# pkuyzy/TLC-GNN

Hardware: AMD Instinct MI355X
Metric: persistence-images/sec + LP-forward edges/sec, PubMed-scale, 1/2/4/8 GPU (higher is better)
Workload: dtype f64; 1 GPU

## Files before the change

tlc-gnn_amd/csrc/ext1_dc.h:

```cpp
#pragma once

#ifndef TLC_DC_MIN_POS
#define TLC_DC_MIN_POS 160
#endif
#ifndef TLC_DC_MIN_POS_SHARED
#define TLC_DC_MIN_POS_SHARED 320
#endif
#define TLC_DC_MAX_TIE_RUN 64

namespace {

struct DcMem {
    unsigned *Qab, *Pab;
    unsigned short *Qseg, *Qw, *Pseg, *Pw, *Phin;
    unsigned* inT;
    unsigned* best;
    unsigned short *comp, *hook, *labL, *labR;
    int S_cap;
};

__host__ __device__ constexpr size_t dc_bytes(int K, int S_cap) {
    return al16((size_t)K * 8) + 5 * al16((size_t)K * 2) + al16((size_t)((2 * K + 31) / 32) * 4) + al16((size_t)S_cap * 4) +
           4 * al16((size_t)S_cap * 2);
}

__device__ __forceinline__ DcMem dc_carve(unsigned char* base, int K, int S_cap) {
    DcMem D;
    size_t o = 0;
    D.Qab = (unsigned*)(base + o);  o += al16((size_t)K * 4);
    D.Pab = (unsigned*)(base + o);  o += al16((size_t)K * 4);
    D.Qseg = (unsigned short*)(base + o); o += al16((size_t)K * 2);
    D.Qw = (unsigned short*)(base + o);   o += al16((size_t)K * 2);
    D.Pseg = (unsigned short*)(base + o); o += al16((size_t)K * 2);
    D.Pw = (unsigned short*)(base + o);   o += al16((size_t)K * 2);
    D.Phin = (unsigned short*)(base + o); o += al16((size_t)K * 2);
    D.inT = (unsigned*)(base + o);  o += al16((size_t)((2 * K + 31) / 32) * 4);
    D.best = (unsigned*)(base + o); o += al16((size_t)S_cap * 4);
    D.comp = (unsigned short*)(base + o); o += al16((size_t)S_cap * 2);
    D.hook = (unsigned short*)(base + o); o += al16((size_t)S_cap * 2);
    D.labL = (unsigned short*)(base + o); o += al16((size_t)S_cap * 2);
    D.labR = (unsigned short*)(base + o); o += al16((size_t)S_cap * 2);
    D.S_cap = S_cap;
    return D;
}

template <int W>
__device__ __forceinline__ int block_exscan_u16(unsigned short* a, int N, int* wcnt) {
    const int tid = threadIdx.x;
    const int per = (N + W - 1) / W;
    const int lo = tid * per, hi = lo + per < N ? lo + per : N;
    int s = 0;
    for (int i = lo; i < hi; ++i) s += a[i];
    const int inc = tlc_wave_iscan_i32(s);
    if (W > 64) {
        if (tlc_lane() == 63) wcnt[tid >> 6] = inc;
        __syncthreads();
    }
    int before = inc - s, total;
    if (W > 64) {
        int t = 0;
#pragma unroll
        for (int k = 0; k < W / 64; ++k) {
            const int c = wcnt[k];
            if (k < (tid >> 6)) before += c;
            t += c;
        }
        total = t;
    } else {
        total = __builtin_amdgcn_readlane(inc, 63);
    }
    for (int i = lo; i < hi; ++i) {
        const int v = a[i];
        a[i] = (unsigned short)before;
        before += v;
    }
    __syncthreads();
    return total;
}

template <int W>
struct AnyFlag {
    int* slots;
    int turn;
    __device__ __forceinline__ void init(int* three_ints) {
        slots = three_ints; turn = 0;
        if (threadIdx.x < 3) slots[threadIdx.x] = 0;
        __syncthreads();
    }
    __device__ __forceinline__ bool any(bool v) {
        if (W == 64) { __syncthreads(); return __ballot(v) != 0ull; }
        const int sl = turn % 3;
        if (v) slots[sl] = 1;
        __syncthreads();
        const bool r = slots[sl] != 0;
        if (threadIdx.x == 0) slots[(sl + 2) % 3] = 0;
        ++turn;
        return r;
    }
};

__device__ __forceinline__ bool dc_jump4(unsigned short* a, int y) {
    const unsigned c = a[y];
    const unsigned p1 = a[c];
    if (p1 == c) return false;
    const unsigned p2 = a[p1];
    const unsigned p3 = a[p2];
    a[y] = (unsigned short)p3;
    return a[p3] != p3;
}
template <int W>
__device__ __forceinline__ void dc_flatten(unsigned short* a, int S, AnyFlag<W>& af) {
    for (int it = 0; it < 32; ++it) {
        bool more = false;
        for (int y = threadIdx.x; y < S; y += W) more |= dc_jump4(a, y);
        if (!af.any(more)) break;
    }
}
template <int W>
__device__ __forceinline__ void dc_flatten2(unsigned short* a, unsigned short* b, int S, AnyFlag<W>& af) {
    for (int it = 0; it < 32; ++it) {
        bool more = false;
        for (int y = threadIdx.x; y < S; y += W) { more |= dc_jump4(a, y); more |= dc_jump4(b, y); }
        if (!af.any(more)) break;
    }
}

template <int W, class ItemsA, class ItemsB>
__device__ __forceinline__ void dc_components2(unsigned short* labA, unsigned short* labB, int S, const ItemsA& itemsA,
                                               const ItemsB& itemsB, AnyFlag<W>& af) {
    const int tid = threadIdx.x;
    for (int x = tid; x < S; x += W) { labA[x] = (unsigned short)x; labB[x] = (unsigned short)x; }
    __syncthreads();
    for (int round = 0; round < 64; ++round) {
        bool ch = false;
        itemsA([&](unsigned ab) {
            const unsigned ra = labA[ab >> 16], rb = labA[ab & 0xffffu];
            if (ra < rb) { labA[rb] = (unsigned short)ra; ch = true; }
            else if (rb < ra) { labA[ra] = (unsigned short)rb; ch = true; }
        });
        itemsB([&](unsigned ab) {
            const unsigned ra = labB[ab >> 16], rb = labB[ab & 0xffffu];
            if (ra < rb) { labB[rb] = (unsigned short)ra; ch = true; }
            else if (rb < ra) { labB[ra] = (unsigned short)rb; ch = true; }
        });
        if (!af.any(ch)) break;
        dc_flatten2<W>(labA, labB, S, af);
    }
}

struct LdsSrc {
    const unsigned *pn, *ends, *arank, *finb;
    int MMcap;
    __device__ __forceinline__ bool neg(int i, unsigned& ab, unsigned& w, bool& fin) const {
        const unsigned e = pn[MMcap - 1 - i];
        ab = ends[e]; w = arank[e]; fin = ((finb[w >> 5] >> (w & 31)) & 1u) != 0u;
        return true;
    }
    __device__ __forceinline__ void pos(int k, unsigned& ab, unsigned& w, bool& fin) const {
        const unsigned e = pn[k];
        ab = ends[e]; w = arank[e]; fin = ((finb[w >> 5] >> (w & 31)) & 1u) != 0u;
    }
};
struct HandoffSrc {
    const unsigned *par, *key;
    const ull* query;
    __device__ __forceinline__ bool neg(int i, unsigned& ab, unsigned& w, bool& fin) const {
        const unsigned k = key[i];
        if (k == 0u) return false;
        const unsigned pr = par[i];
        ab = ((unsigned)i << 16) | (pr & 0xffffu); w = (k >> 8) - 1u; fin = (pr >> 31) != 0u;
        return true;
    }
    __device__ __forceinline__ void pos(int k, unsigned& ab, unsigned& w, bool& fin) const {
        const ull q = query[k];
        ab = (unsigned)q; w = ((unsigned)(q >> 40)) - 1u; fin = ((q >> 32) & 1ull) != 0ull;
    }
};

template <int W, class Src>
__device__ __forceinline__ bool ext1_dc_solve(const Src& src, int n, int K, int n_neg_items, int* ctl, int* wcnt,
                                              unsigned char* scratch, size_t scratch_bytes, unsigned short* out_hin,
                                              unsigned long long* prof = nullptr) {
    const int tid = threadIdx.x;
    unsigned long long t_prev = prof ? clock64() : 0ull;
#define DC_STAMP(k) do { if (prof && tid == 0) { const unsigned long long _t = clock64(); prof[(k)] += _t - t_prev; t_prev = _t; } } while (0)
    const int S_cap = (n > 2 * K + 2 ? n : 2 * K + 2);
    if (K < 2 || K > 16000 || S_cap > 65000 || dc_bytes(K, S_cap) > scratch_bytes) return false;
    const DcMem D = dc_carve(scratch, K, S_cap);
    int* n_pslot = &ctl[10];
    int* bad = &ctl[11];
    if (tid == 0) { *n_pslot = 0; *bad = 0; }
    AnyFlag<W> af;
    af.init(&ctl[12]);
    dc_components2<W>(D.labL, D.labR, n, [&](auto edge) {
        for (int i = tid; i < n_neg_items; i += W) {
            unsigned ab, w; bool fin;
            if (src.neg(i, ab, w, fin) && fin) edge(ab);
        }
    }, [&](auto) {}, af);
    for (int d = tid; d < K; d += W) D.Pseg[d] = 0xFFFFu;
    __syncthreads();
    for (int i = tid; i < n_neg_items; i += W) {
        unsigned ab, w; bool fin;
        if (src.neg(i, ab, w, fin) && !fin) {
            const int d = atomicAdd(n_pslot, 1);
            if (d < K) {
                const unsigned a = ab >> 16, b = ab & 0xffffu;
                D.Pab[d] = ((unsigned)D.labL[a] << 16) | D.labL[b];
                D.Pw[d] = (unsigned short)w;
                D.Phin[d] = (unsigned short)(a > b ? a : b);
                D.Pseg[d] = 0;
            }
        }
    }
    for (int k = tid; k < K; k += W) {
        unsigned ab, w; bool fin;
        src.pos(k, ab, w, fin);
        D.Qab[k] = ((unsigned)D.labL[ab >> 16] << 16) | D.labL[ab & 0xffffu];
        D.Qw[k] = (unsigned short)w;
        D.Qseg[k] = (unsigned short)(fin ? 0x8000u : 0u);
    }
    __syncthreads();
    DC_STAMP(0);
    int S = n;
    int levels = 0;
    while ((1 << levels) < K) ++levels;
    for (int L = 0; L < levels; ++L) {
        const int n_p = *n_pslot < K ? *n_pslot : K;
        auto mid_of = [&](int j) { return (int)(((long long)(2 * j + 1) * K) >> (L + 1)); };
        for (int x = tid; x < S; x += W) D.comp[x] = (unsigned short)x;
        for (int w = tid; w < (2 * K + 31) / 32; w += W) D.inT[w] = 0u;
        __syncthreads();
        for (int round = 0; round < 48; ++round) {
            for (int x = tid; x < S; x += W) { D.best[x] = 0xFFFFFFFFu; D.hook[x] = 0xFFFFu; }
            __syncthreads();
            bool found = false;
            for (int d = tid; d < n_p; d += W) {
                if (D.Pseg[d] == 0xFFFFu) continue;
                const unsigned ab = D.Pab[d];
                const unsigned ra = D.comp[ab >> 16], rb = D.comp[ab & 0xffffu];
                if (ra != rb) {
                    const unsigned key = ((unsigned)D.Pw[d] << 16) | (unsigned)d;
                    atomicMin(&D.best[ra], key); atomicMin(&D.best[rb], key);
                    found = true;
                }
            }
            for (int k = tid; k < K; k += W) {
                if (k >= mid_of(D.Qseg[k] & 0x7FFF)) continue;
                const unsigned ab = D.Qab[k];
                const unsigned ra = D.comp[ab >> 16], rb = D.comp[ab & 0xffffu];
                if (ra != rb) {
                    const unsigned key = ((unsigned)D.Qw[k] << 16) | (unsigned)(K + k);
                    atomicMin(&D.best[ra], key); atomicMin(&D.best[rb], key);
                    found = true;
                }
            }
            if (!af.any(found)) break;
            for (int x = tid; x < S; x += W) {
                const unsigned key = D.best[x];
                if (key == 0xFFFFFFFFu || D.comp[x] != x) continue;
                const int code = (int)(key & 0xffffu);
                const unsigned ab = code < K ? D.Pab[code] : D.Qab[code - K];
                const unsigned ra = D.comp[ab >> 16], rb = D.comp[ab & 0xffffu];
                const unsigned other = (ra == (unsigned)x) ? rb : ra;
                atomicOr(&D.inT[code >> 5], 1u << (code & 31));
                if (D.best[other] != key || (unsigned)x > other) D.hook[x] = (unsigned short)other;
            }
            __syncthreads();
            for (int x = tid; x < S; x += W)
                if (D.hook[x] != 0xFFFFu) D.comp[x] = D.hook[x];
            __syncthreads();
            dc_flatten<W>(D.comp, S, af);
            if (prof && tid == 0) prof[4] += 1;
        }
        DC_STAMP(1);
        auto in_t = [&](int code) { return ((D.inT[code >> 5] >> (code & 31)) & 1u) != 0u; };
        dc_components2<W>(D.labL, D.labR, S, [&](auto edge) {
            for (int d = tid; d < n_p; d += W)
                if (D.Pseg[d] != 0xFFFFu && in_t(d)) edge(D.Pab[d]);
        }, [&](auto edge) {
            for (int k = tid; k < K; k += W) {
                const unsigned sg = D.Qseg[k];
                if (k < mid_of(sg & 0x7FFF) && (sg & 0x8000u) && in_t(K + k)) edge(D.Qab[k]);
            }
        }, af);
        DC_STAMP(2);
        unsigned short* flag = D.comp;
        for (int x = tid; x < 2 * S; x += W) flag[x] = 0;
        __syncthreads();
        auto child_ab = [&](unsigned ab, bool right) -> unsigned {
            const unsigned a = ab >> 16, b = ab & 0xffffu;
            return right ? (((unsigned)(S + D.labR[a]) << 16) | (unsigned)(S + D.labR[b]))
                         : (((unsigned)D.labL[a] << 16) | (unsigned)D.labL[b]);
        };
        for (int d = tid; d < n_p; d += W) {
            if (D.Pseg[d] == 0xFFFFu) continue;
            const unsigned c = child_ab(D.Pab[d], in_t(d));
            flag[c >> 16] = 1; flag[c & 0xffffu] = 1;
        }
        for (int k = tid; k < K; k += W) {
            const bool left = k < mid_of(D.Qseg[k] & 0x7FFF);
            const unsigned c = child_ab(D.Qab[k], !left);
            flag[c >> 16] = 1; flag[c & 0xffffu] = 1;
            if (left && in_t(K + k) && !(D.Qseg[k] & 0x8000u)) {
                const unsigned c2 = child_ab(D.Qab[k], true);
                flag[c2 >> 16] = 1; flag[c2 & 0xffffu] = 1;
            }
        }
        __syncthreads();
        const int S_next = block_exscan_u16<W>(flag, 2 * S, wcnt);
        if (S_next > S_cap) { if (tid == 0) *bad = 1; __syncthreads(); break; }
        auto renum = [&](unsigned c) -> unsigned { return ((unsigned)flag[c >> 16] << 16) | (unsigned)flag[c & 0xffffu]; };
        for (int d = tid; d < n_p; d += W) {
            const unsigned sg = D.Pseg[d];
            if (sg == 0xFFFFu) continue;
            const bool right = in_t(d);
            D.Pab[d] = renum(child_ab(D.Pab[d], right));
            D.Pseg[d] = (unsigned short)(2 * sg + (right ? 1 : 0));
        }
        for (int k = tid; k < K; k += W) {
            const unsigned sg = D.Qseg[k];
            const int j = (int)(sg & 0x7FFF);
            const unsigned ab = D.Qab[k];
            if (k < mid_of(j)) {
                const bool alive_mid = in_t(K + k);
                if (alive_mid && !(sg & 0x8000u)) {
                    const int d = atomicAdd(n_pslot, 1);
                    if (d < K) {
                        D.Pab[d] = renum(child_ab(ab, true));
                        D.Pw[d] = D.Qw[k];
                        { unsigned qab, qw; bool qf; src.pos(k, qab, qw, qf);
                          D.Phin[d] = (unsigned short)((qab >> 16) > (qab & 0xffffu) ? (qab >> 16) : (qab & 0xffffu)); }
                        D.Pseg[d] = (unsigned short)(2 * j + 1);
                    } else *bad = 1;
                }
                D.Qab[k] = renum(child_ab(ab, false));
                D.Qseg[k] = (unsigned short)((2 * j) | (alive_mid ? 0x8000u : 0u));
            } else {
                D.Qab[k] = renum(child_ab(ab, true));
                D.Qseg[k] = (unsigned short)((2 * j + 1) | (sg & 0x8000u));
            }
        }
        __syncthreads();
        S = S_next;
        DC_STAMP(3);
        if (prof && tid == 0) prof[5] += 1;
        if (*bad) break;
    }
    bool fail = (*bad != 0) || (*n_pslot != K);
    __syncthreads();
    if (!fail) {
        for (int w = tid; w < (K + 31) / 32; w += W) D.inT[w] = 0u;
        __syncthreads();
        for (int d = tid; d < K; d += W) {
            const unsigned sg = D.Pseg[d];
            if (sg == 0xFFFFu) { fail = true; continue; }
            const int k = (int)(((long long)sg * K) >> levels);
            const int k1 = (int)(((long long)(sg + 1) * K) >> levels);
            if (k1 - k != 1 || k >= K) { fail = true; continue; }
            const unsigned old = atomicOr(&D.inT[k >> 5], 1u << (k & 31));
            if ((old >> (k & 31)) & 1u) { fail = true; continue; }
            if (D.Pw[d] <= D.Qw[k]) { fail = true; continue; }
            out_hin[k] = D.Phin[d];
        }
        __syncthreads();
    }
#undef DC_STAMP
    return !af.any(fail);
}

template <int W, typename idx_t>
__device__ __forceinline__ bool fix_desc_ties(Mem<idx_t>& M, int m) {
    const int tid = threadIdx.x;
    constexpr int PER = 8;
    int np_[PER];
    unsigned ne_[PER];
    bool too_long = false;
#pragma unroll
    for (int q = 0; q < PER; ++q) {
        const int pos = tid + q * W;
        np_[q] = -1;
        if (pos < m) {
            const ull k = M.keyS[pos];
            const bool tl = pos > 0 && M.keyS[pos - 1] == k, tr = pos + 1 < m && M.keyS[pos + 1] == k;
            if (tl || tr) {
                int s = pos, t = pos + 1;
                while (s > 0 && M.keyS[s - 1] == k && pos - s <= TLC_DC_MAX_TIE_RUN) --s;
                while (t < m && M.keyS[t] == k && t - pos <= TLC_DC_MAX_TIE_RUN) ++t;
                if (t - s > TLC_DC_MAX_TIE_RUN) too_long = true;
                else {
                    const unsigned e = M.valS[pos];
                    const unsigned ar = M.arank[e];
                    int c = 0;
                    for (int j = s; j < t; ++j) c += (M.arank[M.valS[j]] > ar);
                    np_[q] = s + c;
                    ne_[q] = e;
                }
            }
        }
    }
    const bool bad = block_any<W>(too_long, M.ctl, 0);
    if (!bad) {
#pragma unroll
        for (int q = 0; q < PER; ++q)
            if (np_[q] >= 0) M.valS[np_[q]] = ne_[q];
    }
    __syncthreads();
    return !bad;
}

}
```

tlc-gnn_amd/csrc/pd_pipeline.hip:

```cpp
#include "tlc_common.h"
#include "tlc_kernels.h"
#include "pd_keys.h"

#define TLC_INF_BITS 0x7FF0000000000000ull
#ifdef TLC_PHASE_DEBUG
#define TLC_STAMP(k)                                                                 \
    do {                                                                             \
        if (pc && threadIdx.x == 0) {                                                \
            const unsigned long long _t = clock64();                                 \
            ph[(k)] += _t - t_prev;              \
            t_prev = _t;                                                             \
        }                                                                            \
    } while (0)
#else
#define TLC_STAMP(k) do { } while (0)
#endif
#define TLC_NONE16 0xFFFFu
#ifndef TLC_STOP_AFTER
#define TLC_STOP_AFTER 10
#endif
#define TLC_STOPPED 99

namespace {

// ... 1518 lines not shown
        TLC_STAMP(11);
#ifdef TLC_PHASE_DEBUG
        if (pc && tid == 0) {
            const ull tot = clock64() - t_begin;
            for (int k = 0; k < 12; ++k) if (ph[k]) atomicAdd(&pc[k], ph[k]);
            atomicAdd(&pc[12], tot);
            atomicAdd(&pc[14], 1ull);
            if (atomicMax(&pc[13], tot) < tot) {
                for (int k = 0; k < 12; ++k) pc[16 + k] = ph[k];
                pc[28] = (ull)n; pc[29] = (ull)m;
            }
        }
#endif
        if (status != TLC_ST_OK) acc = 0.0;
        if (!deferred) {
            if (p.out_pi && tid < res2) p.out_pi[(size_t)i * res2 + tid] = acc;
            if (p.out_status && tid == 0) p.out_status[i] = (unsigned char)status;
        }
        __syncthreads();
    } while (HUGE && (wi += (int)gridDim.x) < tier_count);
}

struct SwapLayout {
    size_t o_rec, o_pts, o_ctl, total, table_bytes;
};
__host__ __device__ constexpr SwapLayout make_swap_layout(int NM, int MM) {
    SwapLayout L{};
    size_t o = al16(smax(MM <= 1024 ? swap_table_c_bytes(NM) : swap_table_bytes(NM), (size_t)8 * NM + (size_t)64 * 13 * 8));
    L.table_bytes = o - (size_t)8 * NM;
    L.o_rec = o;  o += 1280;
    L.o_pts = o;  o += al16((size_t)(MM + 2) * 4);
    L.o_ctl = o;  o += 64;
    L.total = o;
    return L;
}

template <int NM, int MM, int W>
__device__ __forceinline__ void swap_subgraph(const TlcPdParams& p, int wi, unsigned char* lds_raw) {
    constexpr SwapLayout L = make_swap_layout(NM, MM);
    const int tid = threadIdx.x;
    const Handoff H = carve_handoff(p.handoff + (size_t)wi * (size_t)p.handoff_stride, NM);
    if (H.hdr[0] == 0) return;
    const int i = wi < p.n_hi ? p.tier_list_hi[wi] : p.tier_list[wi - p.n_hi];
    const int n = H.hdr[1], npos = H.hdr[2], np0 = H.hdr[3], n_up = H.hdr[4];
    const bool any_unreached = H.hdr[5] != 0;
    unsigned* pts = (unsigned*)(lds_raw + L.o_pts);
    int* ctl = (int*)(lds_raw + L.o_ctl);
#ifdef TLC_PHASE_DEBUG
    const ull t_begin = clock64();
#endif
    for (int k = tid; k < np0; k += W) pts[k] = H.pts[k];
    PtsSink sink{pts, ctl};
    if constexpr (MM <= 1024) {
        const SwapTablesC T = carve_swap_c(lds_raw, NM);
        unsigned* recs = (unsigned*)(lds_raw + L.o_rec);
        for (int k = tid; k < n; k += W) {
            const unsigned pr = H.par[k];
            T.pk[k] = ((H.key[k] >> 8) << 16) | (pr == 0xffffffffu ? 0xffffu : (pr & 0xffffu));
            T.slot[k] = 0ull;
        }
        if (tid == 0) { T.pk[NM] = (unsigned)NM; T.slot[NM] = 0ull; }
        __syncthreads();
        if (tid < 64) {
            QueryGlobal qs{H.query, npos, 0u, 0u, 0u, 0u, 0u, 0u};
            const int n_out = ext1_walk_c(T, recs, qs, npos, NM, any_unreached, sink, np0);
            if (tid == 0) ctl[2] = np0 + n_out;
        }
    } else {
        const SwapTables T = carve_swap(lds_raw, NM);
        ull* recs = (ull*)(lds_raw + L.o_rec);
        for (int k = tid; k < n; k += W) {
            const unsigned pr = H.par[k];
            T.par[k] = pr == 0xffffffffu ? pr : (pr & 0x7fffffffu);
            T.key[k] = H.key[k];
            T.mark[k] = 0u;
        }
        if (tid == 0) { T.par[NM] = (unsigned)NM; T.key[NM] = 0u; T.mark[NM] = 0u; }
        __syncthreads();
        if (tid < 64) {
            QueryGlobal qs{H.query, npos, 0u, 0u, 0u, 0u, 0u, 0u};
            const int n_out = ext1_walk(T, recs, qs, npos, NM, any_unreached, sink, (const double*)nullptr, false, np0, nullptr);
            if (tid == 0) ctl[2] = np0 + n_out;
        }
    }
    __syncthreads();
    const int np = ctl[2];
    double* f = (double*)lds_raw;
    for (int k = tid; k < n; k += W) f[k] = H.f[k];
    __syncthreads();
    auto get = [&](int k, double& b, double& d) {
        const unsigned bd = pts[k];
        b = f[bd >> 16];
        d = f[bd & 0xffffu];
    };
    const int res = p.res, res2 = res * res;
    double* table = (double*)(lds_raw + (size_t)8 * NM);
    double acc = 0.0;
    if (p.flags & TLC_PI_ORD0_EXT1) {
        acc = pi_stage<W, true, 64>(table, L.table_bytes, get, 0, n_up, res, acc);
        acc = pi_stage<W, true, 64>(table, L.table_bytes, get, n_up + 1, np, res, acc);
    } else {
        acc = pi_stage<W, true, 64>(table, L.table_bytes, get, 0, np, res, acc);
    }
    if (p.out_pi && tid < res2) p.out_pi[(size_t)i * res2 + tid] = acc;
    if (p.out_status && tid == 0) p.out_status[i] = (unsigned char)TLC_ST_OK;
#ifdef TLC_PHASE_DEBUG
    if (p.phase_cycles && tid == 0) { atomicAdd(&p.phase_cycles[10], clock64() - t_begin); atomicAdd(&p.phase_cycles[12], clock64() - t_begin); }
#endif
    __syncthreads();
}

template <int NM, int MM, bool PLAIN = false>
__global__ __launch_bounds__(64, 4) void tlc_pd_swap_kernel(TlcPdParams p) {
    extern __shared__ __attribute__((aligned(16))) unsigned char lds_raw[];
    if constexpr (PLAIN) { p.flags = 0u; p.res = 5; p.pi_enabled = 1; }
    if (p.abort_flag && *p.abort_flag) return;
    int tier_count = p.tier_count;
    if (p.tier_count_dev) { const int c = *p.tier_count_dev; tier_count = c < tier_count ? c : tier_count; }
    if (tier_count > p.handoff_cap) tier_count = p.handoff_cap;
    if ((int)blockIdx.x < tier_count) swap_subgraph<NM, MM, 64>(p, (int)blockIdx.x, lds_raw);
}

__host__ __device__ constexpr size_t dc_kernel_lds(int NM, int MM) {
    const int KB = NM <= TLC_M_NMAX ? (MM / 8) * 7 : MM / 2;
    const size_t dc = al16(dc_bytes(KB, NM > 2 * KB + 2 ? NM : 2 * KB + 2) + (size_t)MM + 16) + al16((size_t)(MM + 2) * 4) + 256;
    return dc > make_swap_layout(NM, MM).total ? dc : make_swap_layout(NM, MM).total;
}
template <int NM, int MM, int W>
__device__ __forceinline__ void dc_subgraph(const TlcPdParams& p, int wi, unsigned char* lds_raw) {
    constexpr size_t total = dc_kernel_lds(NM, MM);
    constexpr size_t o_pts = total - 256 - al16((size_t)(MM + 2) * 4), o_ctl = total - 256;
    const int tid = threadIdx.x;
    unsigned* pts = (unsigned*)(lds_raw + o_pts);
    int* ctl = (int*)(lds_raw + o_ctl);
    int* wcnt = ctl + 16;
    do {
        const Handoff H = carve_handoff(p.handoff + (size_t)wi * (size_t)p.handoff_stride, NM);
        if (H.hdr[0] == 0 || H.hdr[6] == 0) continue;
        const int i = wi < p.n_hi ? p.tier_list_hi[wi] : p.tier_list[wi - p.n_hi];
        const int n = H.hdr[1], K = H.hdr[2], np0 = H.hdr[3], n_up = H.hdr[4];
        const size_t hin_bytes = al16((size_t)K * 2);
        if (hin_bytes + 16 >= o_pts || np0 + K > MM + 2) { __syncthreads(); swap_subgraph<NM, MM, W>(p, wi, lds_raw); continue; }
        unsigned short* hin = (unsigned short*)(lds_raw + (o_pts - hin_bytes));
        const HandoffSrc src{H.par, H.key, H.query};
        __syncthreads();
#ifdef TLC_PHASE_DEBUG
        unsigned long long prof[8] = {0, 0, 0, 0, 0, 0, 0, 0};
        const unsigned long long t_begin = p.phase_cycles ? clock64() : 0ull;
        const bool ok = ext1_dc_solve<W>(src, n, K, n, ctl, wcnt, lds_raw, o_pts - hin_bytes, hin, p.phase_cycles ? prof : nullptr) && !p.dc_force_fail;
        if (p.phase_cycles && tid == 0) {
            const unsigned long long tot = clock64() - t_begin;
            if (atomicMax(&p.phase_cycles[13], tot) < tot) {
                for (int k = 0; k < 6; ++k) p.phase_cycles[16 + k] = prof[k];
                p.phase_cycles[22] = tot; p.phase_cycles[28] = (unsigned long long)n; p.phase_cycles[29] = (unsigned long long)K;
            }
        }
#else
        const bool ok = ext1_dc_solve<W>(src, n, K, n, ctl, wcnt, lds_raw, o_pts - hin_bytes, hin, nullptr) && !p.dc_force_fail;
#endif
        if (!ok) {
            if (p.stats && tid == 0) atomicAdd(&p.stats[3], 1ull);
            __syncthreads();
            swap_subgraph<NM, MM, W>(p, wi, lds_raw);
            continue;
        }
        if (p.stats && tid == 0) atomicAdd(&p.stats[1], 1ull);
        for (int k = tid; k < np0; k += W) pts[k] = H.pts[k];
        for (int k = tid; k < K; k += W) pts[np0 + k] = (((unsigned)(H.query[k] >> 16) & 0xffffu) << 16) | (unsigned)hin[k];
        __syncthreads();
        double* f = (double*)lds_raw;
        for (int k = tid; k < n; k += W) f[k] = H.f[k];
        __syncthreads();
        auto get = [&](int k, double& b, double& d) {
            const unsigned bd = pts[k];
            b = f[bd >> 16];
            d = f[bd & 0xffffu];
        };
        const int res = p.res, res2 = res * res, np = np0 + K;
        double* table = (double*)(lds_raw + al16((size_t)8 * n));
        const size_t table_bytes = (o_pts - hin_bytes) - al16((size_t)8 * n);
        double acc = 0.0;
        if (p.flags & TLC_PI_ORD0_EXT1) {
            acc = pi_stage<W, true, 64>(table, table_bytes, get, 0, n_up, res, acc);
            acc = pi_stage<W, true, 64>(table, table_bytes, get, n_up + 1, np, res, acc);
        } else {
            acc = pi_stage<W, true, 64>(table, table_bytes, get, 0, np, res, acc);
        }
        if (p.out_pi && tid < res2) p.out_pi[(size_t)i * res2 + tid] = acc;
        if (tid == 0) {
            if (p.out_status) p.out_status[i] = (unsigned char)TLC_ST_OK;
            H.hdr[0] = 0;
        }
        __syncthreads();
    } while (false);
}

template <int NM, int MM, int W>
__global__ __launch_bounds__(W, (W <= 256 ? 4 : 1)) void tlc_pd_dc_kernel(TlcPdParams p) {
    extern __shared__ __attribute__((aligned(16))) unsigned char lds_raw[];
    if (p.abort_flag && *p.abort_flag) return;
    int tier_count = p.tier_count;
    if (p.tier_count_dev) { const int c = *p.tier_count_dev; tier_count = c < tier_count ? c : tier_count; }
    if (tier_count > p.handoff_cap) tier_count = p.handoff_cap;
    __builtin_amdgcn_s_setprio(3);
    const int n_list = p.dc_count ? *p.dc_count : 0;
    const int li = blockIdx.x;
    if (li >= n_list) return;
    const int wi = p.dc_list[li];
    if (wi < 0 || wi >= tier_count) return;
    dc_subgraph<NM, MM, W>(p, wi, lds_raw);
}

template <int NM, int MM, int W, bool HUGE>
__global__ __launch_bounds__(W) void tlc_pdf_tier_kernel(TlcPdfParams p) {
    typedef unsigned short idx_t;
    extern __shared__ __attribute__((aligned(16))) unsigned char lds_raw[];
    const int tid = threadIdx.x;
    unsigned char* base;
    Layout L;
    int NMr, MMr;
    if constexpr (HUGE) {
        NMr = p.huge_nmax; MMr = p.huge_mmax;
        L = make_layout(NMr, MMr, sizeof(idx_t), TLC_HUGE_MIN_TABLE);
        base = p.huge_scratch + (size_t)blockIdx.x * p.huge_stride;
    } else {
        NMr = NM; MMr = MM;
        constexpr Layout Lc = make_layout(NM, MM, sizeof(idx_t));
        L = Lc;
        base = lds_raw;
    }
    Mem<idx_t> M = carve<idx_t>(base, L, NMr, MMr);
    int wi = blockIdx.x;
    if (wi >= p.count) return;
    do {
        const int g = p.list[wi];
        const long long no = p.node_offs[g], eo = p.edge_offs[g];
        const int n = (int)(p.node_offs[g + 1] - no), m = (int)(p.edge_offs[g + 1] - eo);
        for (int k = tid; k < n; k += W) M.f[k] = p.f[no + k];
        for (int e = tid; e < m; e += W)
            M.dir[e] = ((unsigned)p.edges[2 * (eo + e)] << 16) | (unsigned)p.edges[2 * (eo + e) + 1];
        if (tid == 0) { M.ctl[2] = 0; M.ctl[3] = 0; M.ctl[4] = 0; M.ctl[6] = 0; M.ctl[7] = 0; M.ctl[8] = 0; }
        __syncthreads();
        GlobalSink sink{p.pd_up + 2 * no, p.pd_down + 2 * no, p.pd_one + 2 * eo, p.ext0 + 2 * (size_t)g, M.ctl};
        ull* pc = nullptr;
        ull t_prev = 0;
        ull* ph = nullptr;
        if (m > 0) {
            bool deferred = false;
            pd_all_stages<W>(M, sink, n, m, p.flags, MMr, NMr, pc, t_prev, ph, nullptr, deferred,
                             (NM == TLC_L_NMAX && !HUGE) ? 1 : 0);
        } else if (tid == 0) {
            double mn = 99999999.0, mx = -99999999.0;
            for (int k = 0; k < n; ++k) { mn = M.f[k] < mn ? M.f[k] : mn; mx = M.f[k] > mx ? M.f[k] : mx; }
            sink.e0[0] = mn; sink.e0[1] = mx;
        }
        __syncthreads();
        const int npos = M.ctl[3], nneg = M.ctl[4];
        if (tid == 0) {
            p.counts[4 * (size_t)g + 0] = M.ctl[6];
            p.counts[4 * (size_t)g + 1] = M.ctl[7];
            p.counts[4 * (size_t)g + 2] = M.ctl[8];
            p.counts[4 * (size_t)g + 3] = n - nneg;
        }
        if (p.edge_rank) {
            for (int k = tid; k < npos; k += W) p.edge_rank[eo + M.pn[k]] = k;
            for (int k = tid; k < nneg; k += W) p.edge_rank[eo + M.pn[MMr - 1 - k]] = -k - 1;
        }
        __syncthreads();
    } while (HUGE && (wi += (int)gridDim.x) < p.count);
}

__global__ void tlc_pdf_bin_kernel(int n_graphs, const long long* node_offs, const long long* edge_offs, int* tier_count,
                                   int* tier_list, int* counts) {
    const int g = blockIdx.x * blockDim.x + threadIdx.x;
    const bool live = g < n_graphs;
    const long long n = live ? node_offs[g + 1] - node_offs[g] : 0, m = live ? edge_offs[g + 1] - edge_offs[g] : 0;
    int tier = TLC_TIER_HUGE;
    if (n <= 0) tier = -1;
    else if (n > TLC_MAX_SUBGRAPH_NODES || m > TLC_MAX_SUBGRAPH_EDGES) {
        tier = -1;
        for (int c = 0; c < 4; ++c) counts[4 * (size_t)g + c] = -1;
    }
    else if (n <= TLC_S_NMAX && m <= TLC_S_MMAX) tier = TLC_TIER_SMALL;
    else if (n <= TLC_M_NMAX && m <= TLC_M_MMAX) tier = TLC_TIER_MEDIUM;
    else if (n <= TLC_L_NMAX && m <= TLC_L_MMAX) tier = TLC_TIER_LARGE;
#pragma unroll
    for (int tt = 0; tt <= TLC_TIER_HUGE; ++tt) {
        const unsigned long long mk = __ballot(tier == tt);
        if (mk == 0ull) continue;
        int base = 0;
        const int leader = __builtin_ctzll(mk);
        if (tlc_lane() == leader) base = atomicAdd(&tier_count[tt], __popcll(mk));
        base = __builtin_amdgcn_readlane(base, leader);
        if (tier == tt) tier_list[(size_t)tt * n_graphs + base + __popcll(mk & tlc_lanemask_lt())] = g;
    }
}

#define TLC_RASTER_MID 96
#define TLC_RASTER_BIG 1024

template <int G>
__device__ __forceinline__ void raster_cdf_row(double base, double step, double (&c)[G], bool& slow) {
    double z[G], t[G], a[G];
#pragma unroll
    for (int g = 0; g < G; ++g) {
        const double zz = ((double)g * step - base) * 0.70710678118654752440;
        const bool in = fabs(zz) <= 0.95;
// ... 422 lines not shown
```

Before: 79.95 million persistence-images/sec.

## Restructure DC level loop: fuse label tracking into MSF rounds, chase pointers, cut barriers

Restructures the per-level divide-and-conquer solve. Component labels for the left and right child are now maintained during the Borůvka MSF rounds by hooking labels alongside comp, and resolved with per-thread pointer chasing instead of iterative flatten passes with barriers. This removes the separate dc_components2 label-propagation pass and the separate flag-marking pass. Relabeling now uses a mark-based exclusive scan followed by one combined renumber pass over P and Q, and loops are unrolled by DC_U to overlap LDS loads. The aim is fewer block-wide barriers and LDS passes per level. In exchange it adds a chase-length cap that can mark a solve bad and force the fallback path, and a new failure flag when the MSF does not converge within 48 rounds.

```diff
diff --git a/tlc-gnn_amd/csrc/ext1_dc.h b/tlc-gnn_amd/csrc/ext1_dc.h
--- a/tlc-gnn_amd/csrc/ext1_dc.h
+++ b/tlc-gnn_amd/csrc/ext1_dc.h
@@ -7,6 +7,10 @@
 #define TLC_DC_MIN_POS_SHARED 320
 #endif
 #define TLC_DC_MAX_TIE_RUN 64
+#ifndef DC_U
+#define DC_U 2
+#endif
+#define DC_CHASE_MAX 1024
 
 namespace {
 
@@ -44,13 +48,13 @@
     return D;
 }
 
-template <int W>
+template <int W, bool MARKS = false>
 __device__ __forceinline__ int block_exscan_u16(unsigned short* a, int N, int* wcnt) {
     const int tid = threadIdx.x;
     const int per = (N + W - 1) / W;
     const int lo = tid * per, hi = lo + per < N ? lo + per : N;
     int s = 0;
-    for (int i = lo; i < hi; ++i) s += a[i];
+    for (int i = lo; i < hi; ++i) s += MARKS ? (a[i] != 0xFFFFu ? 1 : 0) : (int)a[i];
     const int inc = tlc_wave_iscan_i32(s);
     if (W > 64) {
         if (tlc_lane() == 63) wcnt[tid >> 6] = inc;
@@ -70,7 +74,7 @@
         total = __builtin_amdgcn_readlane(inc, 63);
     }
     for (int i = lo; i < hi; ++i) {
-        const int v = a[i];
+        const int v = MARKS ? (a[i] != 0xFFFFu ? 1 : 0) : (int)a[i];
         a[i] = (unsigned short)before;
         before += v;
     }
@@ -107,14 +111,6 @@
     const unsigned p3 = a[p2];
     a[y] = (unsigned short)p3;
     return a[p3] != p3;
-}
-template <int W>
-__device__ __forceinline__ void dc_flatten(unsigned short* a, int S, AnyFlag<W>& af) {
-    for (int it = 0; it < 32; ++it) {
-        bool more = false;
-        for (int y = threadIdx.x; y < S; y += W) more |= dc_jump4(a, y);
-        if (!af.any(more)) break;
-    }
 }
 template <int W>
 __device__ __forceinline__ void dc_flatten2(unsigned short* a, unsigned short* b, int S, AnyFlag<W>& af) {
@@ -184,9 +180,13 @@
     const int tid = threadIdx.x;
     unsigned long long t_prev = prof ? clock64() : 0ull;
 #define DC_STAMP(k) do { if (prof && tid == 0) { const unsigned long long _t = clock64(); prof[(k)] += _t - t_prev; t_prev = _t; } } while (0)
+    int n_bar = 0;
+#define DC_COUNT_BARRIER() do { ++n_bar; } while (0)
+#define DC_BARRIER() do { __syncthreads(); DC_COUNT_BARRIER(); } while (0)
     const int S_cap = (n > 2 * K + 2 ? n : 2 * K + 2);
     if (K < 2 || K > 16000 || S_cap > 65000 || dc_bytes(K, S_cap) > scratch_bytes) return false;
     const DcMem D = dc_carve(scratch, K, S_cap);
+    const unsigned lab_r = (unsigned)(D.labR - D.labL);
     int* n_pslot = &ctl[10];
     int* bad = &ctl[11];
     if (tid == 0) { *n_pslot = 0; *bad = 0; }
@@ -228,125 +228,241 @@
     for (int L = 0; L < levels; ++L) {
         const int n_p = *n_pslot < K ? *n_pslot : K;
         auto mid_of = [&](int j) { return (int)(((long long)(2 * j + 1) * K) >> (L + 1)); };
-        for (int x = tid; x < S; x += W) D.comp[x] = (unsigned short)x;
+        for (int x = tid; x < S; x += W) {
+            D.comp[x] = (unsigned short)x; D.labL[x] = (unsigned short)x; D.labR[x] = (unsigned short)x;
+            D.best[x] = 0xFFFFFFFFu;
+        }
         for (int w = tid; w < (2 * K + 31) / 32; w += W) D.inT[w] = 0u;
-        __syncthreads();
+        DC_BARRIER();
+        bool msf_done = false;
         for (int round = 0; round < 48; ++round) {
-            for (int x = tid; x < S; x += W) { D.best[x] = 0xFFFFFFFFu; D.hook[x] = 0xFFFFu; }
-            __syncthreads();
+            for (int x = tid; x < S; x += W) D.hook[x] = 0xFFFFu;
             bool found = false;
-            for (int d = tid; d < n_p; d += W) {
-                if (D.Pseg[d] == 0xFFFFu) continue;
-                const unsigned ab = D.Pab[d];
-                const unsigned ra = D.comp[ab >> 16], rb = D.comp[ab & 0xffffu];
-                if (ra != rb) {
-                    const unsigned key = ((unsigned)D.Pw[d] << 16) | (unsigned)d;
-                    atomicMin(&D.best[ra], key); atomicMin(&D.best[rb], key);
-                    found = true;
-                }
-            }
-            for (int k = tid; k < K; k += W) {
-                if (k >= mid_of(D.Qseg[k] & 0x7FFF)) continue;
-                const unsigned ab = D.Qab[k];
-                const unsigned ra = D.comp[ab >> 16], rb = D.comp[ab & 0xffffu];
-                if (ra != rb) {
-                    const unsigned key = ((unsigned)D.Qw[k] << 16) | (unsigned)(K + k);
-                    atomicMin(&D.best[ra], key); atomicMin(&D.best[rb], key);
-                    found = true;
-                }
-            }
-            if (!af.any(found)) break;
-            for (int x = tid; x < S; x += W) {
-                const unsigned key = D.best[x];
-                if (key == 0xFFFFFFFFu || D.comp[x] != x) continue;
-                const int code = (int)(key & 0xffffu);
-                const unsigned ab = code < K ? D.Pab[code] : D.Qab[code - K];
-                const unsigned ra = D.comp[ab >> 16], rb = D.comp[ab & 0xffffu];
-                const unsigned other = (ra == (unsigned)x) ? rb : ra;
-                atomicOr(&D.inT[code >> 5], 1u << (code & 31));
-                if (D.best[other] != key || (unsigned)x > other) D.hook[x] = (unsigned short)other;
-            }
-            __syncthreads();
-            for (int x = tid; x < S; x += W)
-                if (D.hook[x] != 0xFFFFu) D.comp[x] = D.hook[x];
-            __syncthreads();
-            dc_flatten<W>(D.comp, S, af);
+            for (int d0 = tid; d0 < n_p; d0 += DC_U * W) {
+                unsigned sg[DC_U], ab[DC_U], wt[DC_U], ra[DC_U], rb[DC_U];
+#pragma unroll
+                for (int q = 0; q < DC_U; ++q) {
+                    const int d = d0 + q * W, dd = d < n_p ? d : 0;
+                    sg[q] = d < n_p ? (unsigned)D.Pseg[dd] : 0xFFFFu; ab[q] = D.Pab[dd]; wt[q] = D.Pw[dd];
+                }
+#pragma unroll
+                for (int q = 0; q < DC_U; ++q) {
+                    if (sg[q] == 0xFFFFu) ab[q] = 0u;
+                    ra[q] = D.comp[ab[q] >> 16]; rb[q] = D.comp[ab[q] & 0xffffu];
+                }
+#pragma unroll
+                for (int q = 0; q < DC_U; ++q)
+                    if (sg[q] != 0xFFFFu && ra[q] != rb[q]) {
+                        const unsigned key = (wt[q] << 16) | (unsigned)(d0 + q * W);
+                        atomicMin(&D.best[ra[q]], key); atomicMin(&D.best[rb[q]], key);
+                        found = true;
+                    }
+            }
+            for (int k0 = tid; k0 < K; k0 += DC_U * W) {
+                unsigned sg[DC_U], ab[DC_U], wt[DC_U], ra[DC_U], rb[DC_U];
+#pragma unroll
+                for (int q = 0; q < DC_U; ++q) {
+                    const int k = k0 + q * W, kk = k < K ? k : 0;
+                    sg[q] = D.Qseg[kk]; ab[q] = D.Qab[kk]; wt[q] = D.Qw[kk];
+                }
+#pragma unroll
+                for (int q = 0; q < DC_U; ++q) { ra[q] = D.comp[ab[q] >> 16]; rb[q] = D.comp[ab[q] & 0xffffu]; }
+#pragma unroll
+                for (int q = 0; q < DC_U; ++q) {
+                    const int k = k0 + q * W;
+                    if (k < K && k < mid_of((int)(sg[q] & 0x7FFFu)) && ra[q] != rb[q]) {
+                        const unsigned key = (wt[q] << 16) | (unsigned)(K + k);
+                        atomicMin(&D.best[ra[q]], key); atomicMin(&D.best[rb[q]], key);
+                        found = true;
+                    }
+                }
+            }
+            DC_COUNT_BARRIER();
+            if (!af.any(found)) { msf_done = true; break; }
+            for (int x0 = tid; x0 < S; x0 += DC_U * W) {
+                unsigned key[DC_U], ab[DC_U], ra[DC_U], rb[DC_U], la[DC_U], lb[DC_U], bo[DC_U];
+                unsigned lab[DC_U];
+                bool joins[DC_U];
+                bool act[DC_U];
+#pragma unroll
+                for (int q = 0; q < DC_U; ++q) {
+                    const int x = x0 + q * W, xx = x < S ? x : 0;
+                    key[q] = D.best[xx];
+                    act[q] = x < S && key[q] != 0xFFFFFFFFu && D.comp[xx] == (unsigned)x;
+                }
+#pragma unroll
+                for (int q = 0; q < DC_U; ++q) {
+                    const int code = act[q] ? (int)(key[q] & 0xffffu) : 0;
+                    const int kq = code < K ? 0 : code - K;
+                    ab[q] = code < K ? D.Pab[code] : D.Qab[kq];
+                    lab[q] = code < K ? 0u : lab_r;
+                    joins[q] = code < K || (D.Qseg[kq] & 0x8000u) != 0u;
+                }
+#pragma unroll
+                for (int q = 0; q < DC_U; ++q) {
+                    const unsigned a = ab[q] >> 16, b = ab[q] & 0xffffu;
+                    ra[q] = D.comp[a]; rb[q] = D.comp[b];
+                    la[q] = D.labL[lab[q] + a]; lb[q] = D.labL[lab[q] + b];
+                }
+#pragma unroll
+                for (int q = 0; q < DC_U; ++q) {
+                    const unsigned x = (unsigned)(x0 + q * W);
+                    if (ra[q] != x) { const unsigned t = ra[q]; ra[q] = rb[q]; rb[q] = t; const unsigned u = la[q]; la[q] = lb[q]; lb[q] = u; }
+                    bo[q] = D.best[act[q] ? rb[q] : 0u];
+                }
+#pragma unroll
+                for (int q = 0; q < DC_U; ++q) {
+                    if (!act[q]) continue;
+                    const unsigned x = (unsigned)(x0 + q * W), other = rb[q];
+                    const int code = (int)(key[q] & 0xffffu);
+                    atomicOr(&D.inT[code >> 5], 1u << (code & 31));
+                    if (bo[q] != key[q] || x > other) {
+                        D.hook[x] = (unsigned short)other;
+                        if (joins[q]) D.labL[lab[q] + la[q]] = (unsigned short)lb[q];
+                    }
+                }
+            }
+            DC_BARRIER();
+            bool lost = false;
+            for (int y0 = tid; y0 < S; y0 += DC_U * W) {
+                unsigned r[DC_U], l[DC_U], m[DC_U];
+#pragma unroll
+                for (int q = 0; q < DC_U; ++q) {
+                    const int y = y0 + q * W, yy = y < S ? y : 0;
+                    r[q] = D.comp[yy]; l[q] = D.labL[yy]; m[q] = D.labR[yy];
+                }
+                for (int it = 0;; ++it) {
+                    unsigned h[DC_U], pl[DC_U], pm[DC_U];
+#pragma unroll
+                    for (int q = 0; q < DC_U; ++q) { h[q] = D.hook[r[q]]; pl[q] = D.labL[l[q]]; pm[q] = D.labR[m[q]]; }
+                    bool moved = false;
+#pragma unroll
+                    for (int q = 0; q < DC_U; ++q) {
+                        if (h[q] != 0xFFFFu) { r[q] = h[q]; moved = true; }
+                        if (pl[q] != l[q]) { l[q] = pl[q]; moved = true; }
+                        if (pm[q] != m[q]) { m[q] = pm[q]; moved = true; }
+                    }
+                    if (!moved) break;
+                    if (it >= DC_CHASE_MAX) { lost = true; break; }
+                }
+#pragma unroll
+                for (int q = 0; q < DC_U; ++q) {
+                    const int y = y0 + q * W;
+                    if (y < S) {
+                        D.comp[y] = (unsigned short)r[q]; D.labL[y] = (unsigned short)l[q]; D.labR[y] = (unsigned short)m[q];
+                        D.best[y] = 0xFFFFFFFFu;
+                    }
+                }
+            }
+            if (lost) *bad = 1;
+            DC_BARRIER();
             if (prof && tid == 0) prof[4] += 1;
         }
+        if (!msf_done) { if (tid == 0) *bad = 1; __syncthreads(); break; }
         DC_STAMP(1);
         auto in_t = [&](int code) { return ((D.inT[code >> 5] >> (code & 31)) & 1u) != 0u; };
-        dc_components2<W>(D.labL, D.labR, S, [&](auto edge) {
-            for (int d = tid; d < n_p; d += W)
-                if (D.Pseg[d] != 0xFFFFu && in_t(d)) edge(D.Pab[d]);
-        }, [&](auto edge) {
-            for (int k = tid; k < K; k += W) {
-                const unsigned sg = D.Qseg[k];
-                if (k < mid_of(sg & 0x7FFF) && (sg & 0x8000u) && in_t(K + k)) edge(D.Qab[k]);
-            }
-        }, af);
+        unsigned short* mark = (unsigned short*)D.best;
+        for (int d0 = tid; d0 < n_p; d0 += DC_U * W) {
+            unsigned sg[DC_U], ab[DC_U], ca[DC_U], cb[DC_U];
+            bool right[DC_U];
+#pragma unroll
+            for (int q = 0; q < DC_U; ++q) {
+                const int d = d0 + q * W, dd = d < n_p ? d : 0;
+                sg[q] = d < n_p ? (unsigned)D.Pseg[dd] : 0xFFFFu; ab[q] = D.Pab[dd]; right[q] = in_t(dd);
+            }
+#pragma unroll
+            for (int q = 0; q < DC_U; ++q) {
+                if (sg[q] == 0xFFFFu) ab[q] = 0u;
+                const unsigned lo = right[q] ? lab_r : 0u;
+                ca[q] = D.labL[lo + (ab[q] >> 16)]; cb[q] = D.labL[lo + (ab[q] & 0xffffu)];
+            }
+#pragma unroll
+            for (int q = 0; q < DC_U; ++q) {
+                if (sg[q] == 0xFFFFu) continue;
+                const int d = d0 + q * W;
+                const unsigned off = right[q] ? (unsigned)S : 0u;
+                ca[q] += off; cb[q] += off;
+                mark[ca[q]] = 0; mark[cb[q]] = 0;
+                D.Pab[d] = (ca[q] << 16) | cb[q];
+                D.Pseg[d] = (unsigned short)(2 * sg[q] + (right[q] ? 1 : 0));
+            }
+        }
+        for (int k0 = tid; k0 < K; k0 += DC_U * W) {
+            unsigned sg[DC_U], ab[DC_U], la[DC_U], lb[DC_U], ra[DC_U], rb[DC_U];
+            bool alive_mid[DC_U];
+#pragma unroll
+            for (int q = 0; q < DC_U; ++q) {
+                const int k = k0 + q * W, kk = k < K ? k : 0;
+                sg[q] = D.Qseg[kk]; ab[q] = D.Qab[kk]; alive_mid[q] = in_t(K + kk);
+            }
+#pragma unroll
+            for (int q = 0; q < DC_U; ++q) {
+                const unsigned a = ab[q] >> 16, b = ab[q] & 0xffffu;
+                la[q] = D.labL[a]; lb[q] = D.labL[b]; ra[q] = (unsigned)S + D.labR[a]; rb[q] = (unsigned)S + D.labR[b];
+            }
+#pragma unroll
+            for (int q = 0; q < DC_U; ++q) {
+                const int k = k0 + q * W;
+                if (k >= K) continue;
+                const int j = (int)(sg[q] & 0x7FFFu);
+                if (k < mid_of(j)) {
+                    if (alive_mid[q] && !(sg[q] & 0x8000u)) {
+                        const int d = atomicAdd(n_pslot, 1);
+                        if (d < K) {
+                            mark[ra[q]] = 0; mark[rb[q]] = 0;
+                            D.Pab[d] = (ra[q] << 16) | rb[q];
+                            D.Pw[d] = D.Qw[k];
+                            { unsigned qab, qw; bool qf; src.pos(k, qab, qw, qf);
+                              D.Phin[d] = (unsigned short)((qab >> 16) > (qab & 0xffffu) ? (qab >> 16) : (qab & 0xffffu)); }
+                            D.Pseg[d] = (unsigned short)(2 * j + 1);
+                        } else *bad = 1;
+                    }
+                    mark[la[q]] = 0; mark[lb[q]] = 0;
+                    D.Qab[k] = (la[q] << 16) | lb[q];
+                    D.Qseg[k] = (unsigned short)((2 * j) | (alive_mid[q] ? 0x8000u : 0u));
+                } else {
+                    mark[ra[q]] = 0; mark[rb[q]] = 0;
+                    D.Qab[k] = (ra[q] << 16) | rb[q];
+                    D.Qseg[k] = (unsigned short)((2 * j + 1) | (sg[q] & 0x8000u));
+                }
+            }
+        }
+        DC_BARRIER();
         DC_STAMP(2);
-        unsigned short* flag = D.comp;
-        for (int x = tid; x < 2 * S; x += W) flag[x] = 0;
-        __syncthreads();
-        auto child_ab = [&](unsigned ab, bool right) -> unsigned {
-            const unsigned a = ab >> 16, b = ab & 0xffffu;
-            return right ? (((unsigned)(S + D.labR[a]) << 16) | (unsigned)(S + D.labR[b]))
-                         : (((unsigned)D.labL[a] << 16) | (unsigned)D.labL[b]);
-        };
-        for (int d = tid; d < n_p; d += W) {
-            if (D.Pseg[d] == 0xFFFFu) continue;
-            const unsigned c = child_ab(D.Pab[d], in_t(d));
-            flag[c >> 16] = 1; flag[c & 0xffffu] = 1;
-        }
-        for (int k = tid; k < K; k += W) {
-            const bool left = k < mid_of(D.Qseg[k] & 0x7FFF);
-            const unsigned c = child_ab(D.Qab[k], !left);
-            flag[c >> 16] = 1; flag[c & 0xffffu] = 1;
-            if (left && in_t(K + k) && !(D.Qseg[k] & 0x8000u)) {
-                const unsigned c2 = child_ab(D.Qab[k], true);
-                flag[c2 >> 16] = 1; flag[c2 & 0xffffu] = 1;
-            }
-        }
-        __syncthreads();
-        const int S_next = block_exscan_u16<W>(flag, 2 * S, wcnt);
+        const int S_next = block_exscan_u16<W, true>(mark, 2 * S, wcnt);
+        DC_COUNT_BARRIER(); if (W > 64) DC_COUNT_BARRIER();
         if (S_next > S_cap) { if (tid == 0) *bad = 1; __syncthreads(); break; }
-        auto renum = [&](unsigned c) -> unsigned { return ((unsigned)flag[c >> 16] << 16) | (unsigned)flag[c & 0xffffu]; };
-        for (int d = tid; d < n_p; d += W) {
-            const unsigned sg = D.Pseg[d];
-            if (sg == 0xFFFFu) continue;
-            const bool right = in_t(d);
-            D.Pab[d] = renum(child_ab(D.Pab[d], right));
-            D.Pseg[d] = (unsigned short)(2 * sg + (right ? 1 : 0));
-        }
-        for (int k = tid; k < K; k += W) {
-            const unsigned sg = D.Qseg[k];
-            const int j = (int)(sg & 0x7FFF);
-            const unsigned ab = D.Qab[k];
-            if (k < mid_of(j)) {
-                const bool alive_mid = in_t(K + k);
-                if (alive_mid && !(sg & 0x8000u)) {
-                    const int d = atomicAdd(n_pslot, 1);
-                    if (d < K) {
-                        D.Pab[d] = renum(child_ab(ab, true));
-                        D.Pw[d] = D.Qw[k];
-                        { unsigned qab, qw; bool qf; src.pos(k, qab, qw, qf);
-                          D.Phin[d] = (unsigned short)((qab >> 16) > (qab & 0xffffu) ? (qab >> 16) : (qab & 0xffffu)); }
-                        D.Pseg[d] = (unsigned short)(2 * j + 1);
-                    } else *bad = 1;
-                }
-                D.Qab[k] = renum(child_ab(ab, false));
-                D.Qseg[k] = (unsigned short)((2 * j) | (alive_mid ? 0x8000u : 0u));
-            } else {
-                D.Qab[k] = renum(child_ab(ab, true));
-                D.Qseg[k] = (unsigned short)((2 * j + 1) | (sg & 0x8000u));
-            }
-        }
-        __syncthreads();
+        const int n_p2 = *n_pslot < K ? *n_pslot : K;
+        for (int i0 = tid; i0 < n_p2 + K; i0 += DC_U * W) {
+            unsigned ab[DC_U], na[DC_U], nb[DC_U];
+            bool on[DC_U];
+#pragma unroll
+            for (int q = 0; q < DC_U; ++q) {
+                const int i = i0 + q * W;
+                const int ii = i < n_p2 ? i : (i < n_p2 + K ? i - n_p2 : 0);
+                on[q] = i < n_p2 ? D.Pseg[ii] != 0xFFFFu : i < n_p2 + K;
+                ab[q] = i < n_p2 ? D.Pab[ii] : D.Qab[ii];
+            }
+#pragma unroll
+            for (int q = 0; q < DC_U; ++q) {
+                if (!on[q]) ab[q] = 0u;
+                na[q] = mark[ab[q] >> 16]; nb[q] = mark[ab[q] & 0xffffu];
+            }
+#pragma unroll
+            for (int q = 0; q < DC_U; ++q) {
+                const int i = i0 + q * W;
+                if (!on[q]) continue;
+                if (i < n_p2) D.Pab[i] = (na[q] << 16) | nb[q];
+                else D.Qab[i - n_p2] = (na[q] << 16) | nb[q];
+            }
+        }
+        DC_BARRIER();
         S = S_next;
         DC_STAMP(3);
         if (prof && tid == 0) prof[5] += 1;
         if (*bad) break;
     }
+    if (prof && tid == 0) prof[6] = (unsigned long long)n_bar;
     bool fail = (*bad != 0) || (*n_pslot != K);
     __syncthreads();
     if (!fail) {
@@ -366,6 +482,8 @@
         __syncthreads();
     }
 #undef DC_STAMP
+#undef DC_BARRIER
+#undef DC_COUNT_BARRIER
     return !af.any(fail);
 }
 
diff --git a/tlc-gnn_amd/csrc/pd_pipeline.hip b/tlc-gnn_amd/csrc/pd_pipeline.hip
--- a/tlc-gnn_amd/csrc/pd_pipeline.hip
+++ b/tlc-gnn_amd/csrc/pd_pipeline.hip
@@ -1694,7 +1694,7 @@
             const unsigned long long tot = clock64() - t_begin;
             if (atomicMax(&p.phase_cycles[13], tot) < tot) {
                 for (int k = 0; k < 6; ++k) p.phase_cycles[16 + k] = prof[k];
-                p.phase_cycles[22] = tot; p.phase_cycles[28] = (unsigned long long)n; p.phase_cycles[29] = (unsigned long long)K;
+                p.phase_cycles[22] = tot; p.phase_cycles[23] = prof[6]; p.phase_cycles[28] = (unsigned long long)n; p.phase_cycles[29] = (unsigned long long)K;
             }
         }
 #else
```

Result: no change. 79.41 million persistence-images/sec (-0.7%).
